# piljoong-jeong/nerf_meets_mlx

Measured on AMD Instinct MI355X. Metric: train+render rays/sec on Lego 800x800 (synthetic), coarse+fine 64+128, higher is better.
Workload: dtype split16 (fp16x2 render / bf16x2 train MFMA operands ~ 22 / 16 significand bits; fp32 accumulate)

## Files before the change

include/nerf_hip.h:

```cpp
#ifndef NERF_HIP_H
#define NERF_HIP_H

#include <stddef.h>
#include <stdint.h>

#ifdef __cplusplus
extern "C" {
#endif

#define NERF_ABI_VERSION 3

#define NERF_OK 0
#define NERF_E_NULL (-1)
#define NERF_E_SHAPE (-2)
#define NERF_E_UNSUPPORTED (-3)
#define NERF_E_HIP (-4)
#define NERF_E_RCCL (-5)

int nerf_abi_version(void);
const char* nerf_last_error(void);

#define NERF_RAY_STRIDE 11

int nerf_pixel_permutation(int64_t* out_idx, int64_t n, int64_t domain, uint64_t seed, uint64_t offset,
// ... 83 lines not shown

typedef struct nerf_mlp_arch {
  int n_layers;
  int width;
  int in_pos;
  int in_dir;
  int skip_layer;
  int use_viewdirs;
  int out_ch;
  int precision;
} nerf_mlp_arch;

int64_t nerf_mlp_param_count(const nerf_mlp_arch* arch);
int64_t nerf_mlp_packed_bytes(const nerf_mlp_arch* arch);
int nerf_mlp_pack(const nerf_mlp_arch* arch, const float* params, void* packed, void* stream);

int64_t nerf_mlp_acts_bytes(const nerf_mlp_arch* arch, int64_t M);
int64_t nerf_mlp_dz_bytes(const nerf_mlp_arch* arch, int64_t M);

int nerf_mlp_forward(const nerf_mlp_arch* arch, const void* packed, const float* x, int64_t M, float* out,
                     void* stream);
int nerf_mlp_forward_train(const nerf_mlp_arch* arch, const void* packed, const float* x, int64_t M, float* out,
                           void* acts, void* stream);

int nerf_query_fused(const nerf_mlp_arch* arch, const void* packed, const float* rays, const float* z, int64_t B,
                     int n, int freq_mode, float* raw, void* acts, void* stream);

int nerf_mlp_backward(const nerf_mlp_arch* arch, const void* packed, const void* acts, const float* d_raw,
                      int64_t M, void* dz, float* grads, void* stream);
int nerf_mlp_backward_inputs(const nerf_mlp_arch* arch, const void* packed, const void* acts, const float* d_raw,
// ... 259 lines not shown
```

nerf_meets_mlx_amd/_native.py:

```python
import ctypes as C
import os

import torch

_HERE = os.path.dirname(os.path.abspath(__file__))
LIB_PATH = os.environ.get("NERF_HIP_LIB", os.path.join(_HERE, "libnerf_hip.so"))

_P, _I64, _I, _F, _U64 = C.c_void_p, C.c_int64, C.c_int, C.c_float, C.c_uint64
SIGNATURES = {
    "nerf_abi_version": (_I, []),
    "nerf_last_error": (C.c_char_p, []),
    "nerf_pixel_permutation": (_I, [_P, _I64, _I64, _U64, _U64, _P]),
    "nerf_ray_gen": (_I, [_P, _I64, _I, _I, C.POINTER(C.c_double), C.POINTER(C.c_float), _F, _F, _P, _P, _P]),
    "nerf_sample_batch": (_I, [_I64, _I, _I, _U64, _U64, C.POINTER(C.c_double), C.POINTER(C.c_float), _F, _F, _P, _P, _P, _P, _P]),
    "nerf_sample_batch_rgba": (_I, [_I64, _I, _I, _U64, _U64, C.POINTER(C.c_double), C.POINTER(C.c_float), _F, _F, _P, _P, _P, _P, _P]),
    "nerf_gather_rows": (_I, [_P, _I64, _P, _I64, _I, _P, _P]),
    "nerf_ndc_rays": (_I, [_P, _I64, _I, _I, _F, _F, _P]),
    "nerf_sample_coarse": (_I, [_P, _I64, _I, _I, _F, _P, _P, _P]),
    "nerf_add_noise_z": (_I, [_P, _P, _I64, _I, _F, _P, _P]),
    "nerf_importance_sample": (_I, [_P, _P, _P, _I64, _I, _I, _F, _P, _P, _P, _P, _P]),
    "nerf_encode_freq": (_I, [_P, _I64, _I, _I, _I, _P, _P]),
    "nerf_encode_sinusoidal": (_I, [_P, _I64, _I, _I, C.POINTER(C.c_float), _I, _P, _P]),
    "nerf_sh_encode": (_I, [_P, _I64, _I, _P, _P]),
    "nerf_hashgrid_forward": (_I, [_P, _I64, _P, _I, _I, _I, C.POINTER(C.c_int), _P, _P]),
# ... 5 lines not shown
    "nerf_hashgrid_backward_ex": (_I, [_P, _I64, _P, _I, _I, _I, C.POINTER(C.c_int), _I, _I, _I, _P, _P]),
    "nerf_hashgrid_backward_rays_ex": (_I, [_P, _P, _I64, _I, _P, _I, _I, _I, C.POINTER(C.c_int), C.c_float, C.c_float, _I, _I, _I, _P, _P]),
    "nerf_hashgrid_forward_lw": (_I, [_P, _I64, _P, _I, _I, _I, C.POINTER(C.c_int), C.POINTER(C.c_float), _P, _P]),
    "nerf_ngp_encode_lw": (_I, [_P, _P, _I64, _I, _P, _I, _I, _I, C.POINTER(C.c_int), C.POINTER(C.c_float), _I, C.c_float, C.c_float, _P, _P, _P]),
    "nerf_ngp_query_fused_lw": (_I, [_P, _P, _P, _P, _I64, _I, _P, _P, _I, _I, _I, C.POINTER(C.c_int), C.POINTER(C.c_float), _I, C.c_float, C.c_float, _P, _P, _P]),
    "nerf_hashgrid_backward_ex_lw": (_I, [_P, _I64, _P, _I, _I, _I, C.POINTER(C.c_int), C.POINTER(C.c_float), _I, _I, _I, _P, _P]),
    "nerf_hashgrid_backward_rays_ex_lw": (_I, [_P, _P, _I64, _I, _P, _I, _I, _I, C.POINTER(C.c_int), C.POINTER(C.c_float), C.c_float, C.c_float, _I, _I, _I, _P, _P]),
    "nerf_composite_forward": (_I, [_P, _P, _P, _I64, _I, _F, _P, _I, _P, _P, _P, _P, _P, _P]),
    "nerf_composite_backward": (_I, [_P, _P, _P, _I64, _I, _F, _P, _I, _P, _P, _P, _P, _P]),
    "nerf_mse_loss_grad": (_I, [_P, _P, _I64, _F, _P, _P, _P]),
    "nerf_composite_mse_backward": (_I, [_P, _P, _P, _I64, _I, _I, _P, _F, _P, _P, _P, _P]),
    "nerf_ssim_sums": (_I, [_P, _P, _I, _I, _I, _I, C.POINTER(C.c_float), _I, _F, _F, _P, _P]),
    "nerf_mlp_param_count": (_I64, [_P]),
    "nerf_mlp_packed_bytes": (_I64, [_P]),
    "nerf_mlp_pack": (_I, [_P, _P, _P, _P]),
    "nerf_mlp_acts_bytes": (_I64, [_P, _I64]),
    "nerf_mlp_dz_bytes": (_I64, [_P, _I64]),
    "nerf_mlp_forward": (_I, [_P, _P, _P, _I64, _P, _P]),
    "nerf_mlp_forward_train": (_I, [_P, _P, _P, _I64, _P, _P, _P]),
    "nerf_query_fused": (_I, [_P, _P, _P, _P, _I64, _I, _I, _P, _P, _P]),
    "nerf_mlp_backward": (_I, [_P, _P, _P, _P, _I64, _P, _P, _P]),
    "nerf_mlp_backward_inputs": (_I, [_P, _P, _P, _P, _I64, _P, _P, _P, _P]),
    "nerf_mlp_debug_width": (_I, [_P, _I, _I]),
    "nerf_mlp_debug_read": (_I, [_P, _P, _I, _I, _I64, _P, _P]),
    "nerf_render_workspace_bytes": (_I64, [_I64, _I, _I]),
    "nerf_render_rays_fused": (_I, [_P, _P, _P, _P, _I64, _I, _I, _P, _I, _I, _P, _P, _P, _P, _P, _P, _P, _P, _P, _P]),
    "nerf_comm_unique_id": (_I, [C.c_char_p]),
    "nerf_comm_init": (_I, [C.POINTER(C.c_void_p), _I, _I, C.c_char_p]),
    "nerf_allreduce_grads": (_I, [_P, _P, _I64, _P]),
    "nerf_comm_destroy": (_I, [_P]),
# ... 158 lines not shown
```

nerf_meets_mlx_amd/csrc/mlp.hip:

```cpp
#include "common.h"
#include "mlp_ring.h"
#include "mlp_layout.h"
#include "mlp_frag.h"
#include "mlp_arch2.h"
#include "mlp_input2.h"
#include "mlp_pack.h"
#include "hash_common.h"
#include "mlp_params.h"
#include "mlp_model.h"
#include "dw_split.h"
#include <limits.h>
#include <string.h>


namespace nerf {

extern int g_hash_combine_max_res;







// ... 234 lines not shown
  pq.init(a.queue, ws.lds0 + Ring::BIAS_OFF);
  for (int64_t sp = blockIdx.x; sp < nsuper;) {
    int ln = lane;
    asm volatile("" : "+v"(ln));
    ws.new_pass();
    fwd_tiles<1, MODE, STORE>(a, ws, sp * NW + wv, ntiles, ln, &pq);
    NERF_STAMP_PASS();
    sp = pq.next(sp);
  }
  NERF_STAMP_END();
  ws.drain();
  pq.leave();
}


constexpr int PACK_BLOCKS = pack_blocks<ViewPack, true>(), PACK16_BLOCKS = L::F16_PADDED * 64 / 256;
__global__ void __launch_bounds__(256) pack_kernel(const float* __restrict__ p, bf16x8* __restrict__ wf,
                                                   bf16x8* __restrict__ wb, float* __restrict__ bias,
                                                   bf16x8* __restrict__ w16) {
  if (blockIdx.x < PACK_BLOCKS) {
    pack_streams<ViewPack, CvtBf16, true>(blockIdx.x * 256 + threadIdx.x, p, wf, wb, bias, 0);
    return;
  }
  const int t = (blockIdx.x - PACK_BLOCKS) * 256 + threadIdx.x;
  if (t >= L::F16_PADDED * 64) return;
  const int f = t >> 6, lane = t & 63;
  bf16x8 v;
#pragma unroll
  for (int j = 0; j < 8; ++j) v[j] = (__bf16)fwd_src16(p, f, lane & 15, lane >> 4, j);
  w16[t] = v;
}

constexpr int RING16_LDS_BYTES = RING_LDS_BYTES;
#ifndef NERF_BF16_IGLP
#define NERF_BF16_IGLP 0
#endif
template <int NS, int KS, int NT, bool RELU, class WS>
__device__ __forceinline__ void layer_fwd16(WS& ws, int fbase, int bias_slot, const bf16x8 (&in)[NS][KS],
                                            bf16x8 (&out)[NS][NT / 2], int lane) {
  const int g = lane >> 4;
  f32x4 prev[NS];
#if NERF_BF16_IGLP >= 0
  __builtin_amdgcn_iglp_opt(NERF_BF16_IGLP);
#endif
  auto finish = [&](int nt, f32x4 (&a)[NS]) {
// ... 791 lines not shown
        }
      }
    }
  }
}

static int g_dw_wgs = 0;
static int g_dw_bias = -1;
static int g_bwd_stage = 0;
static int g_dw_ring_cap = 8;
static int g_dw_private = 4;
static int g_dw16_variant = 1;
static int g_dw_narrow_first = 1;
static int g_dw_factor = 1;
static int g_train_fold = 0;
static int g_dw_job_mask = 0;
static int g_mlp_variant = 0;
static int g_ring_wgs = 0;
static int g_ngp_ray_major = 1;
int g_pass_queue = 1;
static int g_ring_split = 1;

static int cu_count() {
  constexpr int MAX_DEVICES = 64;
  static int n[MAX_DEVICES] = {};
  int dev = 0;
  if (hipGetDevice(&dev) != hipSuccess || dev < 0 || dev >= MAX_DEVICES) dev = 0;
  if (n[dev] == 0) {
    int v = 0;
    n[dev] = (hipDeviceGetAttribute(&v, hipDeviceAttributeMultiprocessorCount, dev) == hipSuccess && v > 0) ? v : 256;
// ... 16 lines not shown
    {"tile_pad16", &g_tile_pad16, opt_clamp<0, INT_MAX>, nullptr},
    {"dw_workgroups", &g_dw_wgs, opt_clamp<0, INT_MAX>, nullptr},
    {"dw_unit_bias", &g_dw_bias, opt_clamp<-1, INT_MAX>, nullptr},
    {"bwd_stage", &g_bwd_stage, opt_any, nullptr},
    {"dw_job_mask", &g_dw_job_mask, opt_any, nullptr},
    {"hash_combine_max_res", &g_hash_combine_max_res, opt_clamp<0, INT_MAX>, nullptr},
    {"ngp_ray_major", &g_ngp_ray_major, opt_flag, nullptr},
    {"dw22_variant", &s16::g_dw_variant, opt_flag, nullptr},
    {"dw16_variant", &g_dw16_variant, opt_clamp<0, 3>, nullptr},
    {"dw_private_tiles", &g_dw_private, opt_clamp<0, 4>, nullptr},
    {"dw_ring_cap", &g_dw_ring_cap, opt_clamp<2, 16>, nullptr},
    {"pass_queue", &g_pass_queue, opt_flag, nullptr},
    {"dw_narrow_first", &g_dw_narrow_first, opt_flag, nullptr},
    {"dw_factor", &g_dw_factor, opt_flag, nullptr},
    {"train_fold", &g_train_fold, opt_flag, nullptr},
    {"f22_tiles", &f22::g_tiles, [](int& v) { return v == 0 || v == 2 || v == 3; }, "nerf_set_option: f22_tiles must be 0 (automatic), 2 or 3"},
};

}

using namespace nerf;

extern "C" int nerf_set_option(const char* key, int value) {
  NERF_REQUIRE(key, NERF_E_NULL, "nerf_set_option: key is NULL");
  NERF_REQUIRE(strcmp(key, "mlp_precision") != 0, NERF_E_UNSUPPORTED,
               "nerf_set_option: \"mlp_precision\" is gone (ABI 3): set nerf_mlp_arch.precision of the model instead");
  for (const Option& o : OPTIONS) {
    if (strcmp(key, o.key)) continue;
    if (!o.rule(value)) return fail(NERF_E_UNSUPPORTED, "%s", o.refusal);
    *o.var = value;
// ... 25 lines not shown
  auto s = as_stream(stream);
  bf16x8* wf = m.stream<bf16x8>(packed, S_FWD);
  bf16x8* wb = m.stream<bf16x8>(packed, S_BWD);
  float* bias = m.stream<float>(packed, S_BIAS);
  int rc;
  if (m.shape == Shape::Small) {
    rc = launch<pack_streams_kernel<SmallPack, CvtBf16, true>>("nerf_mlp_pack (2x64 model)", dim3(pack_blocks<SmallPack, true>()), dim3(256), 0, s,
                                                               params, wf, wb, bias, 0);
    if (!rc && m.split()) rc = s16x::small_pack(params, m.stream<void>(packed, S_S16), s);
  } else if (m.shape == Shape::Image) {
    rc = launch<pack_streams_kernel<ImgPack, CvtBf16, true>>("nerf_mlp_pack (image model)", dim3(pack_blocks<ImgPack, true>()), dim3(256), 0, s,
                                                             params, wf, wb, bias, m.out_ch);
    if (!rc && m.split()) rc = s16x::img_pack(params, m.out_ch, m.stream<void>(packed, S_S16), s);
    if (!rc && m.prec == Prec::F32) rc = f32::pack(params, m.stream<void>(packed, S_F32), m.out_ch, s);
  } else {
    rc = launch<pack_kernel>("nerf_mlp_pack", dim3(PACK_BLOCKS + PACK16_BLOCKS), dim3(256), 0, s, params, wf, wb, bias,
                             m.stream<bf16x8>(packed, S_FWD16));
    if (!rc && m.prec == Prec::F32) rc = f32::pack(params, m.stream<void>(packed, S_F32), 0, s);
    if (!rc && m.split()) rc = f22::pack(params, m.stream<void>(packed, S_F22), s);
    if (!rc && m.split()) rc = s16::pack(params, m.stream<void>(packed, S_S16), train_folded(m), s);
  }
  return rc;
}

template <int MODE>
static int launch_fwd(const Model& m, const void* packed, const float* x, const float* rays, const float* z, int64_t M, int n,
                      int freq_mode, float* out, void* acts, void* stream) {
  FwdArgs a;
  a.queue = nullptr;
  a.wf = m.stream<bf16x8>(packed, S_FWD);
  a.bias = m.stream<float>(packed, S_BIAS);
  a.x = x; a.rays = rays; a.z = z; a.M = M; a.n = n; a.out = out; a.acts = acts; a.astride = m.astride();
  fill_freqs(a.fr.pos, a.fr.dir, freq_mode);
  const int64_t ntiles = (M + 31) / 32;
  auto s = as_stream(stream);
  const int variant = (g_mlp_variant == 0) ? (MODE == 1 ? (acts ? 3 : 4) : 1) : g_mlp_variant;
  if ((variant == 4 || variant == 5) && MODE == 1 && !acts) {
// ... 346 lines not shown
```

nerf_meets_mlx_amd/csrc/mlp22.hip:

```cpp
#include "mlp_layout.h"
#include "mlp22.h"

#ifndef NERF_F22_PIN
#define NERF_F22_PIN 1
#endif
#ifndef NERF_F22_AGPR
#define NERF_F22_AGPR 1
#endif
#ifndef NERF_F22_MIXSUB
#define NERF_F22_MIXSUB 1
#endif
#ifndef NERF_F22_RG3
#define NERF_F22_RG3 4
#endif
#ifndef NERF_F22_PARK
#define NERF_F22_PARK (NERF_F22_FOLD ? 2 : 1)
#endif
#ifndef NERF_F22_IGLP
#define NERF_F22_IGLP 0
#endif

namespace nerf {
namespace f22 {

typedef _Float16 h8 __attribute__((ext_vector_type(8)));
typedef _Float16 h2 __attribute__((ext_vector_type(2)));
typedef float f32x2 __attribute__((ext_vector_type(2)));
typedef unsigned int u32x4 __attribute__((ext_vector_type(4)));

constexpr float LO_SCALE = 2048.0f, LO_INV = 1.0f / 2048.0f;
constexpr float F16_MIN_NORMAL = 6.103515625e-05f;
static_assert(F_CHUNK == RING_CHUNK && CHUNKS == (F_FRAGS + RING_CHUNK - 1) / RING_CHUNK && CHUNKS * RING_CHUNK <= F_PADDED, "f22 ring chunks");
static_assert(P_L0 == L16::F_L0 && P_L1 == L16::F_L1 && P_L5 == L16::F_L5 && P_L6 == L16::F_L6 && P_L7 == L16::F_L7 && P_HEADS == L16::F_FA, "f22 trunk");
#if NERF_F22_FOLD
static_assert(F_PAIRS == L::F16_TOTAL - 128 && CHUNKS == 66 && F_FRAGS % RING_CHUNK == (2 * L::F16_TOTAL) % RING_CHUNK, "f22 folded stream");
#else
static_assert(F_PAIRS == L::F16_TOTAL && P_ALPHA == L16::F_FA + 128 && P_DIR == L16::F_DIR && P_RGB == L16::F_RGB && CHUNKS == 74, "f22 stream layout");
#endif

struct HiLo { unsigned hi, lo; };
__device__ __forceinline__ HiLo split2(float v0, float v1) {
  const f32x2 v = {v0, v1};
  const h2 hh = __builtin_convertvector(v, h2);
#if NERF_F22_MIXSUB
  const f32x2 r = {__builtin_fmaf((float)hh[0], -LO_SCALE, v0 * LO_SCALE), __builtin_fmaf((float)hh[1], -LO_SCALE, v1 * LO_SCALE)};
#else
  const f32x2 r = {(v0 - (float)hh[0]) * LO_SCALE, (v1 - (float)hh[1]) * LO_SCALE};
#endif
  return HiLo{__builtin_bit_cast(unsigned, hh), __builtin_bit_cast(unsigned, __builtin_convertvector(r, h2))};
}

constexpr int PACK_THREADS = (F_PADDED / 2) * 64 + BIAS_FLOATS;
__global__ void __launch_bounds__(256) pack22_kernel(const float* __restrict__ p, u32x4* __restrict__ wf,
                                                     float* __restrict__ bias) {
  const int t = blockIdx.x * 256 + threadIdx.x;
  if (t < (F_PADDED / 2) * 64) {
    const int fp = t >> 6, lane = t & 63;
    u32x4 hi = {0u, 0u, 0u, 0u}, lo = {0u, 0u, 0u, 0u};
    if (fp < F_PAIRS) {
#if NERF_F22_FOLD
      float fold[8] = {0.0f, 0.0f, 0.0f, 0.0f, 0.0f, 0.0f, 0.0f, 0.0f};
      if (fp >= P_DIR && fp < P_RGB && (fp - P_DIR) % 9 < 8) {
        const float* __restrict__ wd = p + L::P_WD + (16 * ((fp - P_DIR) / 9) + (lane & 15)) * 283;
        const float* __restrict__ wfk = p + L::P_WF + kperm16((fp - P_DIR) % 9, lane >> 4, 0);
        double acc[8] = {0.0, 0.0, 0.0, 0.0, 0.0, 0.0, 0.0, 0.0};
#pragma unroll 4
        for (int f = 0; f < 256; ++f) {
          const double a = (double)wd[f];
#pragma unroll
          for (int e = 0; e < 8; ++e) acc[e] = __builtin_fma(a, (double)wfk[f * 256 + 16 * (e >> 2) + (e & 3)], acc[e]);
        }
#pragma unroll
        for (int e = 0; e < 8; ++e) fold[e] = (float)acc[e];
      }
#endif
#pragma unroll
      for (int j = 0; j < 8; j += 2) {
        float w[2];
        _Float16 wh[2], wl[2];
#pragma unroll
        for (int e = 0; e < 2; ++e) {
#if NERF_F22_FOLD
          const Src src = stream_src(fp, lane & 15, lane >> 4, j + e);
          w[e] = src.p >= 0 ? p[src.p] : src.p == SRC_FOLD ? fold[j + e] : 0.0f;
#else
          w[e] = fwd_src16(p, fp, lane & 15, lane >> 4, j + e);
#endif
          wh[e] = __builtin_fabsf(w[e]) < F16_MIN_NORMAL ? (_Float16)0.0f : (_Float16)w[e];
          wl[e] = (_Float16)((w[e] - (float)wh[e]) * LO_SCALE);
        }
        const h2 a = {wh[0], wh[1]}, b = {wl[0], wl[1]};
        hi[j >> 1] = __builtin_bit_cast(unsigned, a);
        lo[j >> 1] = __builtin_bit_cast(unsigned, b);
      }
    }
    wf[(2 * fp) * 64 + lane] = hi;
    wf[(2 * fp + 1) * 64 + lane] = lo;
  } else if (t < PACK_THREADS) {
    const int s = t - (F_PADDED / 2) * 64;
    float v = 0.0f;
    if (s < 2048) v = p[L::pb(s >> 8) + (s & 255)];
#if NERF_F22_FOLD
    else if (s < L::BI_ALPHA) v = 0.0f;
    else if (s < L::BI_DIR) v = (s == L::BI_ALPHA) ? p[L::P_BA] : 0.0f;
    else if (s < L::BI_RGB) {
      const float* __restrict__ wd = p + L::P_WD + (s - L::BI_DIR) * 283;
      double acc = 0.0;
      for (int f = 0; f < 256; ++f) acc = __builtin_fma((double)wd[f], (double)p[L::P_BF + f], acc);
      v = (float)(acc + (double)p[L::P_BD + (s - L::BI_DIR)]);
    }
#else
    else if (s < L::BI_ALPHA) v = p[L::P_BF + (s - L::BI_FEAT)];
    else if (s < L::BI_DIR) v = (s == L::BI_ALPHA) ? p[L::P_BA] : 0.0f;
    else if (s < L::BI_RGB) v = p[L::P_BD + (s - L::BI_DIR)];
#endif
    else v = (s - L::BI_RGB) < 3 ? p[L::P_BR + (s - L::BI_RGB)] : 0.0f;
    bias[s] = v;
  }
}

template <int COUNT>
__device__ __forceinline__ void split_slots(const float (&v)[COUNT], u32x4* hi, u32x4* lo) {
#pragma unroll
  for (int j = 0; j < COUNT; j += 2) {
    const HiLo q = split2(v[j], v[j + 1]);
    hi[j >> 3][(j & 7) >> 1] = q.hi; lo[j >> 3][(j & 7) >> 1] = q.lo;
  }
}
struct SplitF16 {
  static __device__ __forceinline__ void pack(const float (&v)[8], u32x4& hi, u32x4& lo) { split_slots<8>(v, &hi, &lo); }
};

__device__ __forceinline__ f32x4 mfma16(const u32x4& a, const u32x4& b, const f32x4& c) {
// ... 260 lines not shown
  for (int64_t sp = blockIdx.x; sp < nsuper;) {
    int ln = lane;
    asm volatile("" : "+v"(ln));
    ws.new_pass();
    tiles22<NS, MODE>(a, ws, sp * NW22 + wv, nwtiles, ln, pq);
    NERF_STAMP2_PASS();
    sp = pq.next(sp);
  }
  NERF_STAMP2_END();
  ws.drain();
  pq.leave();
}

int pack(const float* params, void* packed22, hipStream_t s) {
  char* base = static_cast<char*>(packed22);
  return launch<pack22_kernel>("nerf_mlp_pack (split-fp16 image)", dim3((PACK_THREADS + 255) / 256), dim3(256), 0, s, params,
                               reinterpret_cast<u32x4*>(base), reinterpret_cast<float*>(base + (size_t)F_PADDED * 1024));
}

int g_tiles = 0;

int forward(const void* packed22, const float* x, const float* rays, const float* z, int64_t M, int n, int freq_mode,
            float* out, int persistent_wgs, hipStream_t s) {
  FwdArgs a;
  a.queue = passq_slot();
  const char* base = static_cast<const char*>(packed22);
  a.wf = reinterpret_cast<const bf16x8*>(base);
  a.bias = reinterpret_cast<const float*>(base + (size_t)F_PADDED * 1024);
  a.x = x; a.rays = rays; a.z = z; a.M = M; a.n = n; a.out = out; a.acts = nullptr; a.astride = 0;
  fill_freqs(a.fr.pos, a.fr.dir, freq_mode);
  int tiles = g_tiles;
// ... 17 lines not shown
```

nerf_meets_mlx_amd/csrc/mlp_s16.hip:

```cpp
#include "mlp_s16_view.h"
#include "mlp_pack.h"

namespace nerf {
namespace s16 {

struct ViewPairPack : ViewPack { static constexpr int B_PADDED = s16::B_PADDED / 2; };
static_assert(ViewPairPack::B_PADDED >= L::B_TOTAL, "the padded stream holds every transposed fragment");

#ifndef NERF_DWX
#define NERF_DWX 0
#endif
#if NERF_DWX & 4
#define DW_BARRIER() do {} while (0)
#else
#define DW_BARRIER() __builtin_amdgcn_s_barrier()
#endif
constexpr int DW_WAVES = 16, DW_NPW = 2;

__device__ __forceinline__ bf16x8 tr_pair(const char* blk, int hq, int fsel, int i16) {
  const int q = i16 >> 2, p = i16 & 3;
  const char* base = blk + 64 * (8 * hq + q) + 32 * fsel + 16 * (p & 1) + 8 * (p >> 1);
#if NERF_DWX & 2
  bf16x8 r; asm volatile("" : "=v"(r) : "v"(base)); return r;
#endif
// ... 361 lines not shown
```

nerf_meets_mlx_amd/csrc/mlp_s16f.hip:

```cpp
#include "mlp_s16_view.h"

namespace nerf {
namespace s16 {

constexpr int FOLD_PACK_PAIRS = (LF::F_TOTAL + LF::B_PADDED) * 64;
constexpr int FOLD_PACK_THREADS = FOLD_PACK_PAIRS + (LF::C_WFT_END - LF::C_WFT) + (LF::C_END - LF::C_WD1);
__global__ void __launch_bounds__(256) pack_fold_kernel(const float* __restrict__ p, bf16x8* __restrict__ img) {
  const int tid = blockIdx.x * 256 + threadIdx.x;
  bf16x8* wf = img;
  bf16x8* wb = img + (size_t)F_FRAGS * 64;
  float* cp = reinterpret_cast<float*>(img);
  if (tid < FOLD_PACK_PAIRS) {
    const bool fw = tid < LF::F_TOTAL * 64;
    const int t = fw ? tid : tid - LF::F_TOTAL * 64;
    const int f = t >> 6, lane = t & 63, r = lane & 31, h = lane >> 5;
    int src[8];
#pragma unroll
    for (int j = 0; j < 8; ++j) src[j] = !fw && f >= LF::B_TOTAL ? -1 : fw ? fwd_index_fold(f, r, h, j) : bwd_index_fold(f, r, h, j);
    const bool wp = is_fold_wp(src[0]);
    if (wp && !fw) return;
    float v[8];
    if (wp) {
      const int n = fold_wp_n(src[0]);
      double acc[8];
#pragma unroll
      for (int j = 0; j < 8; ++j) acc[j] = 0.0;
      for (int q = 0; q < 256; ++q) {
        const double wd = (double)p[L::P_WD + n * 283 + q];
#pragma unroll
        for (int j = 0; j < 8; ++j) acc[j] = __builtin_fma(wd, (double)p[L::P_WF + q * 256 + fold_wp_k(src[j])], acc[j]);
      }
#pragma unroll
      for (int j = 0; j < 8; ++j) v[j] = (float)acc[j];
    } else {
#pragma unroll
      for (int j = 0; j < 8; ++j) v[j] = src[j] >= 0 ? p[src[j]] : 0.0f;
    }
    bf16x8 o[2];
    SplitBf16::pack(v, o[0], o[1]);
    bf16x8* dst = fw ? wf : wb;
    dst[(2 * f) * 64 + lane] = o[0];
    dst[(2 * f + 1) * 64 + lane] = o[1];
    if (wp) {
      __bf16* tb = reinterpret_cast<__bf16*>(wb);
#pragma unroll
      for (int j = 0; j < 8; ++j) {
        const FragElem e = fold_elem_bwd(fold_wp_n(src[j]), fold_wp_k(src[j]));
        FragElem eh = e, el = e;
        eh.f = 2 * e.f; el.f = 2 * e.f + 1;
        tb[frag_elem_offset(eh)] = o[0][j];
        tb[frag_elem_offset(el)] = o[1][j];
      }
    }
    return;
  }
  int c = tid - FOLD_PACK_PAIRS;
  if (c < LF::C_WFT_END - LF::C_WFT) {
    cp[LF::C_WFT + c] = p[L::P_WF + (c & 255) * 256 + (c >> 8)];
    return;
  }
  c += LF::C_WD1 - (LF::C_WFT_END - LF::C_WFT);
  if (c >= LF::C_END) return;
  float v = 0.0f;
  if (c < LF::C_BF) { const int e = c - LF::C_WD1; v = p[L::P_WD + (e >> 8) * 283 + (e & 255)]; }
  else if (c < LF::C_BP) v = p[L::P_BF + (c - LF::C_BF)];
  else if (c < LF::C_USED) {
    const int n = c - LF::C_BP;
    double acc = 0.0;
    for (int q = 0; q < 256; ++q) acc = __builtin_fma((double)p[L::P_WD + n * 283 + q], (double)p[L::P_BF + q], acc);
    v = (float)(acc + (double)p[L::P_BD + n]);
  }
  cp[c] = v;
}

int pack_folded(const float* params, void* packed_s16, hipStream_t s) {
  return launch<pack_fold_kernel>("nerf_mlp_pack (split-bf16 image, folded)", dim3((FOLD_PACK_THREADS + 255) / 256), dim3(256), 0, s, params,
                                  static_cast<bf16x8*>(packed_s16));
}

int forward_folded(const void* packed_s16, const float* bias_slots, const float* x, const float* rays, const float* z, int64_t M,
                   int n, int freq_mode, float* out, void* acts, int64_t astride16, int persistent_wgs, hipStream_t s) {
  FwdArgs a;
  a.queue = passq_slot();
  a.wf = reinterpret_cast<const bf16x8*>(packed_s16);
  a.bias = bias_slots;
  a.x = x; a.rays = rays; a.z = z; a.M = M; a.n = n; a.out = out; a.acts = acts; a.astride = astride16;
  fill_freqs(a.fr.pos, a.fr.dir, freq_mode);
  const int64_t nsuper = ((M + 31) / 32 + NW - 1) / NW;
  return with_bool(x != nullptr, [&](auto rows) {
    return launch<s16_fwd_kernel<decltype(rows)::value ? 0 : 1, true>>("mlp training forward (split bf16, folded)",
                                                                        dim3(persistent_grid(nsuper, persistent_wgs)), dim3(64 * NW),
// ... 18 lines not shown
```

Measured before the change: 1.350 million.

## Share folded weight product across pack streams and pack in one launch

```diff
diff --git a/include/nerf_hip.h b/include/nerf_hip.h
--- a/include/nerf_hip.h
+++ b/include/nerf_hip.h
@@ -121,6 +121,7 @@
 int64_t nerf_mlp_param_count(const nerf_mlp_arch* arch);
 int64_t nerf_mlp_packed_bytes(const nerf_mlp_arch* arch);
 int nerf_mlp_pack(const nerf_mlp_arch* arch, const float* params, void* packed, void* stream);
+int nerf_mlp_fold_product(const nerf_mlp_arch* arch, const float* params, float* w_out, float* b_out, void* stream);
 
 int64_t nerf_mlp_acts_bytes(const nerf_mlp_arch* arch, int64_t M);
 int64_t nerf_mlp_dz_bytes(const nerf_mlp_arch* arch, int64_t M);
diff --git a/nerf_meets_mlx_amd/_native.py b/nerf_meets_mlx_amd/_native.py
--- a/nerf_meets_mlx_amd/_native.py
+++ b/nerf_meets_mlx_amd/_native.py
@@ -43,6 +43,7 @@
     "nerf_mlp_param_count": (_I64, [_P]),
     "nerf_mlp_packed_bytes": (_I64, [_P]),
     "nerf_mlp_pack": (_I, [_P, _P, _P, _P]),
+    "nerf_mlp_fold_product": (_I, [_P, _P, _P, _P, _P]),
     "nerf_mlp_acts_bytes": (_I64, [_P, _I64]),
     "nerf_mlp_dz_bytes": (_I64, [_P, _I64]),
     "nerf_mlp_forward": (_I, [_P, _P, _P, _I64, _P, _P]),
diff --git a/nerf_meets_mlx_amd/csrc/mlp.hip b/nerf_meets_mlx_amd/csrc/mlp.hip
--- a/nerf_meets_mlx_amd/csrc/mlp.hip
+++ b/nerf_meets_mlx_amd/csrc/mlp.hip
@@ -4,7 +4,7 @@
 #include "mlp_frag.h"
 #include "mlp_arch2.h"
 #include "mlp_input2.h"
-#include "mlp_pack.h"
+#include "mlp_pack_view.h"
 #include "hash_common.h"
 #include "mlp_params.h"
 #include "mlp_model.h"
@@ -272,21 +272,10 @@
 }
 
 
-constexpr int PACK_BLOCKS = pack_blocks<ViewPack, true>(), PACK16_BLOCKS = L::F16_PADDED * 64 / 256;
 __global__ void __launch_bounds__(256) pack_kernel(const float* __restrict__ p, bf16x8* __restrict__ wf,
                                                    bf16x8* __restrict__ wb, float* __restrict__ bias,
                                                    bf16x8* __restrict__ w16) {
-  if (blockIdx.x < PACK_BLOCKS) {
-    pack_streams<ViewPack, CvtBf16, true>(blockIdx.x * 256 + threadIdx.x, p, wf, wb, bias, 0);
-    return;
-  }
-  const int t = (blockIdx.x - PACK_BLOCKS) * 256 + threadIdx.x;
-  if (t >= L::F16_PADDED * 64) return;
-  const int f = t >> 6, lane = t & 63;
-  bf16x8 v;
-#pragma unroll
-  for (int j = 0; j < 8; ++j) v[j] = (__bf16)fwd_src16(p, f, lane & 15, lane >> 4, j);
-  w16[t] = v;
+  pack_view_bf16(blockIdx.x, p, wf, wb, bias, w16);
 }
 
 constexpr int RING16_LDS_BYTES = RING_LDS_BYTES;
@@ -1108,6 +1097,7 @@
 static int g_dw_narrow_first = 1;
 static int g_dw_factor = 1;
 static int g_train_fold = 0;
+static int g_pack_shared = 1;
 static int g_dw_job_mask = 0;
 static int g_mlp_variant = 0;
 static int g_ring_wgs = 0;
@@ -1154,6 +1144,7 @@
     {"dw_narrow_first", &g_dw_narrow_first, opt_flag, nullptr},
     {"dw_factor", &g_dw_factor, opt_flag, nullptr},
     {"train_fold", &g_train_fold, opt_flag, nullptr},
+    {"pack_shared", &g_pack_shared, opt_flag, nullptr},
     {"f22_tiles", &f22::g_tiles, [](int& v) { return v == 0 || v == 2 || v == 3; }, "nerf_set_option: f22_tiles must be 0 (automatic), 2 or 3"},
 };
 
@@ -1209,6 +1200,15 @@
     if (!rc && m.split()) rc = s16x::img_pack(params, m.out_ch, m.stream<void>(packed, S_S16), s);
     if (!rc && m.prec == Prec::F32) rc = f32::pack(params, m.stream<void>(packed, S_F32), m.out_ch, s);
   } else {
+    if (m.split() && g_pack_shared) {
+      const bool fold = train_folded(m), need = NERF_F22_FOLD || fold;
+      float* wp = need ? foldw::scratch(s) : nullptr;
+      if (wp || !need) {
+        if (need) NERF_TRY(foldw::product(params, wp, s));
+        return foldw::pack_view_split({params, wp, wf, wb, m.stream<void>(packed, S_FWD16), bias, m.stream<void>(packed, S_F22),
+                                       m.stream<void>(packed, S_S16)}, fold, s);
+      }
+    }
     rc = launch<pack_kernel>("nerf_mlp_pack", dim3(PACK_BLOCKS + PACK16_BLOCKS), dim3(256), 0, s, params, wf, wb, bias,
                              m.stream<bf16x8>(packed, S_FWD16));
     if (!rc && m.prec == Prec::F32) rc = f32::pack(params, m.stream<void>(packed, S_F32), 0, s);
@@ -1216,6 +1216,20 @@
     if (!rc && m.split()) rc = s16::pack(params, m.stream<void>(packed, S_S16), train_folded(m), s);
   }
   return rc;
+}
+
+extern "C" int nerf_mlp_fold_product(const nerf_mlp_arch* arch, const float* params, float* w_out, float* b_out, void* stream) {
+  NERF_RESOLVE("nerf_mlp_fold_product");
+  NERF_REQUIRE(m.can_factor(), NERF_E_UNSUPPORTED, "nerf_mlp_fold_product: only the 8 x 256 view model at precision 22 folds its feature layer");
+  NERF_REQUIRE(params && w_out && b_out, NERF_E_NULL, "nerf_mlp_fold_product: NULL pointer");
+  auto s = as_stream(stream);
+  float* wp = foldw::scratch(s);
+  NERF_REQUIRE(wp, NERF_E_HIP, "nerf_mlp_fold_product: no scratch for this stream (capturing, more than 64 streams, or out of memory)");
+  NERF_TRY(foldw::product(params, wp, s));
+  if (hipMemcpyAsync(w_out, wp, sizeof(float) * foldw::WP_FLOATS, hipMemcpyDeviceToDevice, s) != hipSuccess ||
+      hipMemcpyAsync(b_out, wp + foldw::WP_FLOATS, sizeof(float) * foldw::N, hipMemcpyDeviceToDevice, s) != hipSuccess)
+    return fail(NERF_E_HIP, "nerf_mlp_fold_product: copy out of the scratch failed");
+  return NERF_OK;
 }
 
 template <int MODE>
diff --git a/nerf_meets_mlx_amd/csrc/mlp22.hip b/nerf_meets_mlx_amd/csrc/mlp22.hip
--- a/nerf_meets_mlx_amd/csrc/mlp22.hip
+++ b/nerf_meets_mlx_amd/csrc/mlp22.hip
@@ -1,5 +1,6 @@
 #include "mlp_layout.h"
 #include "mlp22.h"
+#include "mlp_pack_view.h"
 
 #ifndef NERF_F22_PIN
 #define NERF_F22_PIN 1
@@ -24,12 +25,8 @@
 namespace f22 {
 
 typedef _Float16 h8 __attribute__((ext_vector_type(8)));
-typedef _Float16 h2 __attribute__((ext_vector_type(2)));
 typedef float f32x2 __attribute__((ext_vector_type(2)));
-typedef unsigned int u32x4 __attribute__((ext_vector_type(4)));
-
-constexpr float LO_SCALE = 2048.0f, LO_INV = 1.0f / 2048.0f;
-constexpr float F16_MIN_NORMAL = 6.103515625e-05f;
+
 static_assert(F_CHUNK == RING_CHUNK && CHUNKS == (F_FRAGS + RING_CHUNK - 1) / RING_CHUNK && CHUNKS * RING_CHUNK <= F_PADDED, "f22 ring chunks");
 static_assert(P_L0 == L16::F_L0 && P_L1 == L16::F_L1 && P_L5 == L16::F_L5 && P_L6 == L16::F_L6 && P_L7 == L16::F_L7 && P_HEADS == L16::F_FA, "f22 trunk");
 #if NERF_F22_FOLD
@@ -50,73 +47,9 @@
   return HiLo{__builtin_bit_cast(unsigned, hh), __builtin_bit_cast(unsigned, __builtin_convertvector(r, h2))};
 }
 
-constexpr int PACK_THREADS = (F_PADDED / 2) * 64 + BIAS_FLOATS;
 __global__ void __launch_bounds__(256) pack22_kernel(const float* __restrict__ p, u32x4* __restrict__ wf,
                                                      float* __restrict__ bias) {
-  const int t = blockIdx.x * 256 + threadIdx.x;
-  if (t < (F_PADDED / 2) * 64) {
-    const int fp = t >> 6, lane = t & 63;
-    u32x4 hi = {0u, 0u, 0u, 0u}, lo = {0u, 0u, 0u, 0u};
-    if (fp < F_PAIRS) {
-#if NERF_F22_FOLD
-      float fold[8] = {0.0f, 0.0f, 0.0f, 0.0f, 0.0f, 0.0f, 0.0f, 0.0f};
-      if (fp >= P_DIR && fp < P_RGB && (fp - P_DIR) % 9 < 8) {
-        const float* __restrict__ wd = p + L::P_WD + (16 * ((fp - P_DIR) / 9) + (lane & 15)) * 283;
-        const float* __restrict__ wfk = p + L::P_WF + kperm16((fp - P_DIR) % 9, lane >> 4, 0);
-        double acc[8] = {0.0, 0.0, 0.0, 0.0, 0.0, 0.0, 0.0, 0.0};
-#pragma unroll 4
-        for (int f = 0; f < 256; ++f) {
-          const double a = (double)wd[f];
-#pragma unroll
-          for (int e = 0; e < 8; ++e) acc[e] = __builtin_fma(a, (double)wfk[f * 256 + 16 * (e >> 2) + (e & 3)], acc[e]);
-        }
-#pragma unroll
-        for (int e = 0; e < 8; ++e) fold[e] = (float)acc[e];
-      }
-#endif
-#pragma unroll
-      for (int j = 0; j < 8; j += 2) {
-        float w[2];
-        _Float16 wh[2], wl[2];
-#pragma unroll
-        for (int e = 0; e < 2; ++e) {
-#if NERF_F22_FOLD
-          const Src src = stream_src(fp, lane & 15, lane >> 4, j + e);
-          w[e] = src.p >= 0 ? p[src.p] : src.p == SRC_FOLD ? fold[j + e] : 0.0f;
-#else
-          w[e] = fwd_src16(p, fp, lane & 15, lane >> 4, j + e);
-#endif
-          wh[e] = __builtin_fabsf(w[e]) < F16_MIN_NORMAL ? (_Float16)0.0f : (_Float16)w[e];
-          wl[e] = (_Float16)((w[e] - (float)wh[e]) * LO_SCALE);
-        }
-        const h2 a = {wh[0], wh[1]}, b = {wl[0], wl[1]};
-        hi[j >> 1] = __builtin_bit_cast(unsigned, a);
-        lo[j >> 1] = __builtin_bit_cast(unsigned, b);
-      }
-    }
-    wf[(2 * fp) * 64 + lane] = hi;
-    wf[(2 * fp + 1) * 64 + lane] = lo;
-  } else if (t < PACK_THREADS) {
-    const int s = t - (F_PADDED / 2) * 64;
-    float v = 0.0f;
-    if (s < 2048) v = p[L::pb(s >> 8) + (s & 255)];
-#if NERF_F22_FOLD
-    else if (s < L::BI_ALPHA) v = 0.0f;
-    else if (s < L::BI_DIR) v = (s == L::BI_ALPHA) ? p[L::P_BA] : 0.0f;
-    else if (s < L::BI_RGB) {
-      const float* __restrict__ wd = p + L::P_WD + (s - L::BI_DIR) * 283;
-      double acc = 0.0;
-      for (int f = 0; f < 256; ++f) acc = __builtin_fma((double)wd[f], (double)p[L::P_BF + f], acc);
-      v = (float)(acc + (double)p[L::P_BD + (s - L::BI_DIR)]);
-    }
-#else
-    else if (s < L::BI_ALPHA) v = p[L::P_BF + (s - L::BI_FEAT)];
-    else if (s < L::BI_DIR) v = (s == L::BI_ALPHA) ? p[L::P_BA] : 0.0f;
-    else if (s < L::BI_RGB) v = p[L::P_BD + (s - L::BI_DIR)];
-#endif
-    else v = (s - L::BI_RGB) < 3 ? p[L::P_BR + (s - L::BI_RGB)] : 0.0f;
-    bias[s] = v;
-  }
+  pack22_body<false>(blockIdx.x * 256 + threadIdx.x, p, nullptr, wf, bias);
 }
 
 template <int COUNT>
@@ -407,7 +340,7 @@
 
 int pack(const float* params, void* packed22, hipStream_t s) {
   char* base = static_cast<char*>(packed22);
-  return launch<pack22_kernel>("nerf_mlp_pack (split-fp16 image)", dim3((PACK_THREADS + 255) / 256), dim3(256), 0, s, params,
+  return launch<pack22_kernel>("nerf_mlp_pack (split-fp16 image)", dim3(PACK22_BLOCKS), dim3(256), 0, s, params,
                                reinterpret_cast<u32x4*>(base), reinterpret_cast<float*>(base + (size_t)F_PADDED * 1024));
 }
 
diff --git a/nerf_meets_mlx_amd/csrc/mlp_foldw.h b/nerf_meets_mlx_amd/csrc/mlp_foldw.h
--- /dev/null
+++ b/nerf_meets_mlx_amd/csrc/mlp_foldw.h
@@ -0,0 +1,42 @@
+#pragma once
+#ifdef __HIPCC__
+#include <hip/hip_runtime.h>
+#endif
+#include <stdint.h>
+#include "mlp_index.h"
+
+namespace nerf {
+namespace foldw {
+
+constexpr int N = 128, K = 256, J = 256;
+constexpr int WP_FLOATS = N * K, SCRATCH_FLOATS = WP_FLOATS + N;
+__host__ __device__ constexpr int wp_at(int n, int k) { return n * K + k; }
+__host__ __device__ constexpr int bp_at(int n) { return WP_FLOATS + n; }
+
+constexpr int TILE_N = 4, TILE_K = 32, THREADS = TILE_N * TILE_K;
+constexpr int W_BLOCKS = (N / TILE_N) * (K / TILE_K), B_BLOCKS = N / TILE_N, BLOCKS = W_BLOCKS + B_BLOCKS;
+static_assert(N % TILE_N == 0 && K % TILE_K == 0 && THREADS % 64 == 0, "whole tiles, whole waves");
+struct Tile { int n0, k0; };
+__host__ __device__ constexpr Tile tile_of(int block) {
+  return block < W_BLOCKS ? Tile{TILE_N * (block / (K / TILE_K)), TILE_K * (block % (K / TILE_K))} : Tile{TILE_N * (block - W_BLOCKS), -1};
+}
+__host__ __device__ constexpr int product_dst(int block, int t) {
+  const Tile tl = tile_of(block);
+  const int r = t / TILE_K, c = t % TILE_K;
+  if (tl.k0 < 0) return c == 0 ? bp_at(tl.n0 + r) : -1;
+  return wp_at(tl.n0 + r, tl.k0 + c);
+}
+
+#ifdef __HIPCC__
+float* scratch(hipStream_t s);
+int product(const float* params, float* scratch, hipStream_t s);
+struct PackViewArgs {
+  const float* p; const float* wp;
+  void *wf, *wb, *w16; float* bias;
+  void* f22; void* s16;
+};
+int pack_view_split(const PackViewArgs& a, bool fold, hipStream_t s);
+#endif
+
+}
+}
diff --git a/nerf_meets_mlx_amd/csrc/mlp_foldw.hip b/nerf_meets_mlx_amd/csrc/mlp_foldw.hip
--- /dev/null
+++ b/nerf_meets_mlx_amd/csrc/mlp_foldw.hip
@@ -0,0 +1,92 @@
+#include "common.h"
+#include "launch.h"
+#include "mlp_pack_view.h"
+
+namespace nerf {
+namespace foldw {
+
+__global__ void __launch_bounds__(THREADS) fold_product_kernel(const float* __restrict__ p, float* __restrict__ scratch) {
+  __shared__ float wf_s[J][TILE_K];
+  __shared__ float wd_s[TILE_N][J];
+  const Tile tl = tile_of(blockIdx.x);
+  const int t = threadIdx.x;
+  constexpr int WD_PER = TILE_N * J / THREADS, WF_PER = J * TILE_K / THREADS, BF_PER = J / THREADS;
+  float wd_r[WD_PER], wf_r[WF_PER];
+#pragma unroll
+  for (int m = 0; m < WD_PER; ++m) { const int i = t + m * THREADS; wd_r[m] = p[L::P_WD + (tl.n0 + i / J) * 283 + i % J]; }
+  if (tl.k0 >= 0) {
+#pragma unroll
+    for (int m = 0; m < WF_PER; ++m) { const int i = t + m * THREADS; wf_r[m] = p[L::P_WF + (i / TILE_K) * K + tl.k0 + i % TILE_K]; }
+#pragma unroll
+    for (int m = 0; m < WF_PER; ++m) { const int i = t + m * THREADS; wf_s[i / TILE_K][i % TILE_K] = wf_r[m]; }
+  } else {
+#pragma unroll
+    for (int m = 0; m < BF_PER; ++m) wf_r[m] = p[L::P_BF + t + m * THREADS];
+#pragma unroll
+    for (int m = 0; m < BF_PER; ++m) wf_s[t + m * THREADS][0] = wf_r[m];
+  }
+#pragma unroll
+  for (int m = 0; m < WD_PER; ++m) { const int i = t + m * THREADS; wd_s[i / J][i % J] = wd_r[m]; }
+  __syncthreads();
+  const int r = t / TILE_K, c = t % TILE_K;
+  const int dst = product_dst(blockIdx.x, t);
+  if (dst < 0) return;
+  double acc = 0.0;
+#pragma unroll 8
+  for (int j = 0; j < J; ++j) acc = __builtin_fma((double)wd_s[r][j], (double)wf_s[j][c], acc);
+  scratch[dst] = tl.k0 >= 0 ? (float)acc : (float)(acc + (double)p[L::P_BD + tl.n0 + r]);
+}
+
+int product(const float* params, float* scratch, hipStream_t s) {
+  return launch<fold_product_kernel>("nerf_mlp_pack (folded product)", dim3(BLOCKS), dim3(THREADS), 0, s, params, scratch);
+}
+
+constexpr int BF16_BLOCKS = PACK_BLOCKS + PACK16_BLOCKS, F22_END = BF16_BLOCKS + f22::PACK22_BLOCKS;
+constexpr int S16_BLOCKS = pack_blocks<s16::ViewPairPack, false>();
+template <bool FOLD>
+__global__ void __launch_bounds__(256) pack_view_split_kernel(PackViewArgs a) {
+  const int b = blockIdx.x;
+  if (b < BF16_BLOCKS) {
+    pack_view_bf16(b, a.p, static_cast<bf16x8*>(a.wf), static_cast<bf16x8*>(a.wb), a.bias, static_cast<bf16x8*>(a.w16));
+  } else if (b < F22_END) {
+    char* base = static_cast<char*>(a.f22);
+    f22::pack22_body<true>((b - BF16_BLOCKS) * 256 + threadIdx.x, a.p, a.wp, reinterpret_cast<f22::u32x4*>(base),
+                           reinterpret_cast<float*>(base + (size_t)f22::F_PADDED * 1024));
+  } else {
+    const int tid = (b - F22_END) * 256 + threadIdx.x;
+    bf16x8* img = static_cast<bf16x8*>(a.s16);
+    if constexpr (FOLD) s16::pack_fold_body<true>(tid, a.p, a.wp, img);
+    else pack_streams<s16::ViewPairPack, s16::SplitBf16, false>(tid, a.p, img, img + (size_t)s16::F_FRAGS * 64, nullptr, 0);
+  }
+}
+
+int pack_view_split(const PackViewArgs& a, bool fold, hipStream_t s) {
+  return with_bool(fold, [&](auto f) {
+    constexpr bool FOLD = decltype(f)::value;
+    return launch<pack_view_split_kernel<FOLD>>("nerf_mlp_pack (precision 22, one launch)",
+                                                dim3(F22_END + (FOLD ? s16::FOLD_PACK_BLOCKS : S16_BLOCKS)), dim3(256), 0, s, a);
+  });
+}
+
+float* scratch(hipStream_t s) {
+  constexpr int SLOTS = 64;
+  struct Slot { int dev; hipStream_t stream; float* buf; };
+  static Slot slots[SLOTS];
+  static int used = 0;
+  static std::mutex mu;
+  const int dev = DevOnce::device();
+  std::lock_guard<std::mutex> lock(mu);
+  for (int i = 0; i < used; ++i)
+    if (slots[i].dev == dev && slots[i].stream == s) return slots[i].buf;
+  if (used == SLOTS) return nullptr;
+  hipStreamCaptureStatus cap = hipStreamCaptureStatusNone;
+  if (hipStreamIsCapturing(s, &cap) != hipSuccess) { (void)hipGetLastError(); return nullptr; }
+  if (cap != hipStreamCaptureStatusNone) return nullptr;
+  void* buf = nullptr;
+  if (hipMalloc(&buf, sizeof(float) * SCRATCH_FLOATS) != hipSuccess) { (void)hipGetLastError(); return nullptr; }
+  slots[used++] = Slot{dev, s, static_cast<float*>(buf)};
+  return slots[used - 1].buf;
+}
+
+}
+}
diff --git a/nerf_meets_mlx_amd/csrc/mlp_pack_view.h b/nerf_meets_mlx_amd/csrc/mlp_pack_view.h
--- /dev/null
+++ b/nerf_meets_mlx_amd/csrc/mlp_pack_view.h
@@ -0,0 +1,198 @@
+#pragma once
+#include "mlp_pack.h"
+#include "mlp22.h"
+#include "mlp_s16.h"
+#include "mlp_s16_dev.h"
+#include "mlp_foldw.h"
+
+namespace nerf {
+
+constexpr int PACK_BLOCKS = pack_blocks<ViewPack, true>(), PACK16_BLOCKS = L::F16_PADDED * 64 / 256;
+__device__ __forceinline__ void pack_view_bf16(int block, const float* __restrict__ p, bf16x8* __restrict__ wf, bf16x8* __restrict__ wb,
+                                               float* __restrict__ bias, bf16x8* __restrict__ w16) {
+  if (block < PACK_BLOCKS) {
+    pack_streams<ViewPack, CvtBf16, true>(block * 256 + threadIdx.x, p, wf, wb, bias, 0);
+    return;
+  }
+  const int t = (block - PACK_BLOCKS) * 256 + threadIdx.x;
+  if (t >= L::F16_PADDED * 64) return;
+  const int f = t >> 6, lane = t & 63;
+  bf16x8 v;
+#pragma unroll
+  for (int j = 0; j < 8; ++j) v[j] = (__bf16)fwd_src16(p, f, lane & 15, lane >> 4, j);
+  w16[t] = v;
+}
+
+namespace f22 {
+
+typedef _Float16 h2 __attribute__((ext_vector_type(2)));
+typedef unsigned int u32x4 __attribute__((ext_vector_type(4)));
+constexpr float LO_SCALE = 2048.0f, LO_INV = 1.0f / 2048.0f;
+constexpr float F16_MIN_NORMAL = 6.103515625e-05f;
+
+constexpr int PACK_THREADS = (F_PADDED / 2) * 64 + BIAS_FLOATS, PACK22_BLOCKS = (PACK_THREADS + 255) / 256;
+template <bool SHARED>
+__device__ __forceinline__ void pack22_body(int t, const float* __restrict__ p, const float* __restrict__ wp, u32x4* __restrict__ wf,
+                                            float* __restrict__ bias) {
+  if (t < (F_PADDED / 2) * 64) {
+    const int fp = t >> 6, lane = t & 63;
+    u32x4 hi = {0u, 0u, 0u, 0u}, lo = {0u, 0u, 0u, 0u};
+    if (fp < F_PAIRS) {
+#if NERF_F22_FOLD
+      float fold[8] = {0.0f, 0.0f, 0.0f, 0.0f, 0.0f, 0.0f, 0.0f, 0.0f};
+      if (fp >= P_DIR && fp < P_RGB && (fp - P_DIR) % 9 < 8) {
+        const int n = 16 * ((fp - P_DIR) / 9) + (lane & 15), k0 = kperm16((fp - P_DIR) % 9, lane >> 4, 0);
+        if constexpr (SHARED) {
+#pragma unroll
+          for (int e = 0; e < 8; ++e) fold[e] = wp[foldw::wp_at(n, k0 + 16 * (e >> 2) + (e & 3))];
+        } else {
+          const float* __restrict__ wd = p + L::P_WD + n * 283;
+          const float* __restrict__ wfk = p + L::P_WF + k0;
+          double acc[8] = {0.0, 0.0, 0.0, 0.0, 0.0, 0.0, 0.0, 0.0};
+#pragma unroll 4
+          for (int f = 0; f < 256; ++f) {
+            const double a = (double)wd[f];
+#pragma unroll
+            for (int e = 0; e < 8; ++e) acc[e] = __builtin_fma(a, (double)wfk[f * 256 + 16 * (e >> 2) + (e & 3)], acc[e]);
+          }
+#pragma unroll
+          for (int e = 0; e < 8; ++e) fold[e] = (float)acc[e];
+        }
+      }
+#endif
+#pragma unroll
+      for (int j = 0; j < 8; j += 2) {
+        float w[2];
+        _Float16 wh[2], wl[2];
+#pragma unroll
+        for (int e = 0; e < 2; ++e) {
+#if NERF_F22_FOLD
+          const Src src = stream_src(fp, lane & 15, lane >> 4, j + e);
+          w[e] = src.p >= 0 ? p[src.p] : src.p == SRC_FOLD ? fold[j + e] : 0.0f;
+#else
+          w[e] = fwd_src16(p, fp, lane & 15, lane >> 4, j + e);
+#endif
+          wh[e] = __builtin_fabsf(w[e]) < F16_MIN_NORMAL ? (_Float16)0.0f : (_Float16)w[e];
+          wl[e] = (_Float16)((w[e] - (float)wh[e]) * LO_SCALE);
+        }
+        const h2 a = {wh[0], wh[1]}, b = {wl[0], wl[1]};
+        hi[j >> 1] = __builtin_bit_cast(unsigned, a);
+        lo[j >> 1] = __builtin_bit_cast(unsigned, b);
+      }
+    }
+    wf[(2 * fp) * 64 + lane] = hi;
+    wf[(2 * fp + 1) * 64 + lane] = lo;
+  } else if (t < PACK_THREADS) {
+    const int s = t - (F_PADDED / 2) * 64;
+    float v = 0.0f;
+    if (s < 2048) v = p[L::pb(s >> 8) + (s & 255)];
+#if NERF_F22_FOLD
+    else if (s < L::BI_ALPHA) v = 0.0f;
+    else if (s < L::BI_DIR) v = (s == L::BI_ALPHA) ? p[L::P_BA] : 0.0f;
+    else if (s < L::BI_RGB) {
+      if constexpr (SHARED) v = wp[foldw::bp_at(s - L::BI_DIR)];
+      else {
+        const float* __restrict__ wd = p + L::P_WD + (s - L::BI_DIR) * 283;
+        double acc = 0.0;
+        for (int f = 0; f < 256; ++f) acc = __builtin_fma((double)wd[f], (double)p[L::P_BF + f], acc);
+        v = (float)(acc + (double)p[L::P_BD + (s - L::BI_DIR)]);
+      }
+    }
+#else
+    else if (s < L::BI_ALPHA) v = p[L::P_BF + (s - L::BI_FEAT)];
+    else if (s < L::BI_DIR) v = (s == L::BI_ALPHA) ? p[L::P_BA] : 0.0f;
+    else if (s < L::BI_RGB) v = p[L::P_BD + (s - L::BI_DIR)];
+#endif
+    else v = (s - L::BI_RGB) < 3 ? p[L::P_BR + (s - L::BI_RGB)] : 0.0f;
+    bias[s] = v;
+  }
+}
+
+}
+
+namespace s16 {
+
+struct ViewPairPack : ViewPack { static constexpr int B_PADDED = s16::B_PADDED / 2; };
+static_assert(ViewPairPack::B_PADDED >= L::B_TOTAL, "the padded stream holds every transposed fragment");
+
+constexpr int FOLD_PACK_PAIRS = (LF::F_TOTAL + LF::B_PADDED) * 64;
+constexpr int FOLD_PACK_THREADS = FOLD_PACK_PAIRS + (LF::C_WFT_END - LF::C_WFT) + (LF::C_END - LF::C_WD1);
+constexpr int FOLD_PACK_BLOCKS = (FOLD_PACK_THREADS + 255) / 256;
+template <bool SHARED>
+__device__ __forceinline__ void pack_fold_body(int tid, const float* __restrict__ p, const float* __restrict__ wp, bf16x8* __restrict__ img) {
+  bf16x8* wf = img;
+  bf16x8* wb = img + (size_t)F_FRAGS * 64;
+  float* cp = reinterpret_cast<float*>(img);
+  if (tid < FOLD_PACK_PAIRS) {
+    const bool fw = tid < LF::F_TOTAL * 64;
+    const int t = fw ? tid : tid - LF::F_TOTAL * 64;
+    const int f = t >> 6, lane = t & 63, r = lane & 31, h = lane >> 5;
+    int src[8];
+#pragma unroll
+    for (int j = 0; j < 8; ++j) src[j] = !fw && f >= LF::B_TOTAL ? -1 : fw ? fwd_index_fold(f, r, h, j) : bwd_index_fold(f, r, h, j);
+    const bool wpe = is_fold_wp(src[0]);
+    if (!SHARED && wpe && !fw) return;
+    float v[8];
+    if (wpe) {
+      if constexpr (SHARED) {
+#pragma unroll
+        for (int j = 0; j < 8; ++j) v[j] = wp[foldw::wp_at(fold_wp_n(src[j]), fold_wp_k(src[j]))];
+      } else {
+        const int n = fold_wp_n(src[0]);
+        double acc[8];
+#pragma unroll
+        for (int j = 0; j < 8; ++j) acc[j] = 0.0;
+        for (int q = 0; q < 256; ++q) {
+          const double wd = (double)p[L::P_WD + n * 283 + q];
+#pragma unroll
+          for (int j = 0; j < 8; ++j) acc[j] = __builtin_fma(wd, (double)p[L::P_WF + q * 256 + fold_wp_k(src[j])], acc[j]);
+        }
+#pragma unroll
+        for (int j = 0; j < 8; ++j) v[j] = (float)acc[j];
+      }
+    } else {
+#pragma unroll
+      for (int j = 0; j < 8; ++j) v[j] = src[j] >= 0 ? p[src[j]] : 0.0f;
+    }
+    bf16x8 o[2];
+    SplitBf16::pack(v, o[0], o[1]);
+    bf16x8* dst = fw ? wf : wb;
+    dst[(2 * f) * 64 + lane] = o[0];
+    dst[(2 * f + 1) * 64 + lane] = o[1];
+    if (!SHARED && wpe) {
+      __bf16* tb = reinterpret_cast<__bf16*>(wb);
+#pragma unroll
+      for (int j = 0; j < 8; ++j) {
+        const FragElem e = fold_elem_bwd(fold_wp_n(src[j]), fold_wp_k(src[j]));
+        FragElem eh = e, el = e;
+        eh.f = 2 * e.f; el.f = 2 * e.f + 1;
+        tb[frag_elem_offset(eh)] = o[0][j];
+        tb[frag_elem_offset(el)] = o[1][j];
+      }
+    }
+    return;
+  }
+  int c = tid - FOLD_PACK_PAIRS;
+  if (c < LF::C_WFT_END - LF::C_WFT) {
+    cp[LF::C_WFT + c] = p[L::P_WF + (c & 255) * 256 + (c >> 8)];
+    return;
+  }
+  c += LF::C_WD1 - (LF::C_WFT_END - LF::C_WFT);
+  if (c >= LF::C_END) return;
+  float v = 0.0f;
+  if (c < LF::C_BF) { const int e = c - LF::C_WD1; v = p[L::P_WD + (e >> 8) * 283 + (e & 255)]; }
+  else if (c < LF::C_BP) v = p[L::P_BF + (c - LF::C_BF)];
+  else if (c < LF::C_USED) {
+    const int n = c - LF::C_BP;
+    if constexpr (SHARED) v = wp[foldw::bp_at(n)];
+    else {
+      double acc = 0.0;
+      for (int q = 0; q < 256; ++q) acc = __builtin_fma((double)p[L::P_WD + n * 283 + q], (double)p[L::P_BF + q], acc);
+      v = (float)(acc + (double)p[L::P_BD + n]);
+    }
+  }
+  cp[c] = v;
+}
+
+}
+}
diff --git a/nerf_meets_mlx_amd/csrc/mlp_s16.hip b/nerf_meets_mlx_amd/csrc/mlp_s16.hip
--- a/nerf_meets_mlx_amd/csrc/mlp_s16.hip
+++ b/nerf_meets_mlx_amd/csrc/mlp_s16.hip
@@ -1,11 +1,9 @@
 #include "mlp_s16_view.h"
-#include "mlp_pack.h"
+#include "mlp_pack_view.h"
 
 namespace nerf {
 namespace s16 {
 
-struct ViewPairPack : ViewPack { static constexpr int B_PADDED = s16::B_PADDED / 2; };
-static_assert(ViewPairPack::B_PADDED >= L::B_TOTAL, "the padded stream holds every transposed fragment");
 
 #ifndef NERF_DWX
 #define NERF_DWX 0
diff --git a/nerf_meets_mlx_amd/csrc/mlp_s16f.hip b/nerf_meets_mlx_amd/csrc/mlp_s16f.hip
--- a/nerf_meets_mlx_amd/csrc/mlp_s16f.hip
+++ b/nerf_meets_mlx_amd/csrc/mlp_s16f.hip
@@ -1,80 +1,15 @@
 #include "mlp_s16_view.h"
+#include "mlp_pack_view.h"
 
 namespace nerf {
 namespace s16 {
 
-constexpr int FOLD_PACK_PAIRS = (LF::F_TOTAL + LF::B_PADDED) * 64;
-constexpr int FOLD_PACK_THREADS = FOLD_PACK_PAIRS + (LF::C_WFT_END - LF::C_WFT) + (LF::C_END - LF::C_WD1);
 __global__ void __launch_bounds__(256) pack_fold_kernel(const float* __restrict__ p, bf16x8* __restrict__ img) {
-  const int tid = blockIdx.x * 256 + threadIdx.x;
-  bf16x8* wf = img;
-  bf16x8* wb = img + (size_t)F_FRAGS * 64;
-  float* cp = reinterpret_cast<float*>(img);
-  if (tid < FOLD_PACK_PAIRS) {
-    const bool fw = tid < LF::F_TOTAL * 64;
-    const int t = fw ? tid : tid - LF::F_TOTAL * 64;
-    const int f = t >> 6, lane = t & 63, r = lane & 31, h = lane >> 5;
-    int src[8];
-#pragma unroll
-    for (int j = 0; j < 8; ++j) src[j] = !fw && f >= LF::B_TOTAL ? -1 : fw ? fwd_index_fold(f, r, h, j) : bwd_index_fold(f, r, h, j);
-    const bool wp = is_fold_wp(src[0]);
-    if (wp && !fw) return;
-    float v[8];
-    if (wp) {
-      const int n = fold_wp_n(src[0]);
-      double acc[8];
-#pragma unroll
-      for (int j = 0; j < 8; ++j) acc[j] = 0.0;
-      for (int q = 0; q < 256; ++q) {
-        const double wd = (double)p[L::P_WD + n * 283 + q];
-#pragma unroll
-        for (int j = 0; j < 8; ++j) acc[j] = __builtin_fma(wd, (double)p[L::P_WF + q * 256 + fold_wp_k(src[j])], acc[j]);
-      }
-#pragma unroll
-      for (int j = 0; j < 8; ++j) v[j] = (float)acc[j];
-    } else {
-#pragma unroll
-      for (int j = 0; j < 8; ++j) v[j] = src[j] >= 0 ? p[src[j]] : 0.0f;
-    }
-    bf16x8 o[2];
-    SplitBf16::pack(v, o[0], o[1]);
-    bf16x8* dst = fw ? wf : wb;
-    dst[(2 * f) * 64 + lane] = o[0];
-    dst[(2 * f + 1) * 64 + lane] = o[1];
-    if (wp) {
-      __bf16* tb = reinterpret_cast<__bf16*>(wb);
-#pragma unroll
-      for (int j = 0; j < 8; ++j) {
-        const FragElem e = fold_elem_bwd(fold_wp_n(src[j]), fold_wp_k(src[j]));
-        FragElem eh = e, el = e;
-        eh.f = 2 * e.f; el.f = 2 * e.f + 1;
-        tb[frag_elem_offset(eh)] = o[0][j];
-        tb[frag_elem_offset(el)] = o[1][j];
-      }
-    }
-    return;
-  }
-  int c = tid - FOLD_PACK_PAIRS;
-  if (c < LF::C_WFT_END - LF::C_WFT) {
-    cp[LF::C_WFT + c] = p[L::P_WF + (c & 255) * 256 + (c >> 8)];
-    return;
-  }
-  c += LF::C_WD1 - (LF::C_WFT_END - LF::C_WFT);
-  if (c >= LF::C_END) return;
-  float v = 0.0f;
-  if (c < LF::C_BF) { const int e = c - LF::C_WD1; v = p[L::P_WD + (e >> 8) * 283 + (e & 255)]; }
-  else if (c < LF::C_BP) v = p[L::P_BF + (c - LF::C_BF)];
-  else if (c < LF::C_USED) {
-    const int n = c - LF::C_BP;
-    double acc = 0.0;
-    for (int q = 0; q < 256; ++q) acc = __builtin_fma((double)p[L::P_WD + n * 283 + q], (double)p[L::P_BF + q], acc);
-    v = (float)(acc + (double)p[L::P_BD + n]);
-  }
-  cp[c] = v;
+  pack_fold_body<false>(blockIdx.x * 256 + threadIdx.x, p, nullptr, img);
 }
 
 int pack_folded(const float* params, void* packed_s16, hipStream_t s) {
-  return launch<pack_fold_kernel>("nerf_mlp_pack (split-bf16 image, folded)", dim3((FOLD_PACK_THREADS + 255) / 256), dim3(256), 0, s, params,
+  return launch<pack_fold_kernel>("nerf_mlp_pack (split-bf16 image, folded)", dim3(FOLD_PACK_BLOCKS), dim3(256), 0, s, params,
                                   static_cast<bf16x8*>(packed_s16));
 }
 
```

Result: no change. 1.349 million, median of 2 (-0.0%).
